# aleju/cat-generator

Measured on AMD Instinct MI355X. Metric: images/sec per G+D step, G32up-c 32x32 RGB bs=128 per GPU, higher is better.
Workload: dtype f32

## Files before the change

cat-generator_amd/csrc/common.h:

```cpp
#pragma once
#include <hip/hip_runtime.h>
#include <algorithm>
#include <stdint.h>
#include <stdio.h>
#include <string.h>
#include "../../include/catgan.h"

namespace cg {

char* err_buf();
int fail(const char* fmt, ...);

inline hipStream_t S(void* s) { return reinterpret_cast<hipStream_t>(s); }

#define CG_HIP(call)                                                              \
    do {                                                                          \
        hipError_t e__ = (call);                                                  \
        if (e__ != hipSuccess)                                                    \
            return cg::fail("%s:%d %s -> %s", __FILE__, __LINE__, #call,          \
                            hipGetErrorString(e__));                              \
    } while (0)

#define CG_LAUNCH_CHECK()                                                         \
    do {                                                                          \
        hipError_t e__ = hipGetLastError();                                       \
        if (e__ != hipSuccess)                                                    \
            return cg::fail("%s:%d kernel launch -> %s", __FILE__, __LINE__,      \
                            hipGetErrorString(e__));                              \
    } while (0)

#define CG_REQUIRE(cond, ...)                                                     \
    do {                                                                          \
        if (!(cond)) return cg::fail(__VA_ARGS__);                                \
    } while (0)

constexpr int kNumCU = 256;

#ifndef CG_TIMING_PROBE
#define CG_TIMING_PROBE 0
#endif
#define CG_PROBE_HALF(fam, T) (((CG_TIMING_PROBE) & (fam)) ? ((T) + 1) / 2 : (T))
constexpr int kEwWgsPerCU = 4, kColReduceWgsPerCU = 1;

enum Opt {
    OPT_SKINNY, OPT_GEMM_BK32, OPT_WINO_BK, OPT_NN_TILE, OPT_TN_TILE, OPT_NN_SPLITS, OPT_TN_SPLITS,
    OPT_XCD_SWIZZLE, OPT_NN_GLDS, OPT_TN_GLDS, OPT_WINO_GLDS, OPT_PAD_SKIP, OPT_WINO3, OPT_COUNT
};
long opt(Opt o);

static inline int cdiv(long a, long b) { return (int)((a + b - 1) / b); }

constexpr size_t kColScratchBytes = 8u << 20;
void* col_scratch(hipStream_t stream);
hipStream_t queue_stream(hipStream_t ref, int cls, int slot);
int queue_class(hipStream_t ref, hipStream_t s);
void wgrad_discard_all();

constexpr int kSkinnyWgradBlocks = 512;
bool skinny_ok(int ngroups, int Cin, int Cout, int kH, int kW, int padH, int padW, int ups);
size_t skinny_wgrad_ws_bytes(int Cin, int Cout);
void skinny_valu_forward(hipStream_t st, const float* x, const float* w, const float* bias, float* y, int N, int H, int W, int Cin, int Cout);
void skinny_valu_wgrad(hipStream_t st, const float* x, const float* dy, float* part, float* bias_part, int N, int H, int W, int Cin, int Cout,
                       int blocks, long ppb);
bool skinny_mfma_ok(int Cin, int Cout, int H, int W);
int skinny_mfma_forward(hipStream_t st, const float* x, const float* w, const float* bias, float* y, int N, int H, int W, int Cin, int Cout);
int skinny_mfma_wgrad(hipStream_t st, const float* x, const float* dy, float* part, float* bias_part, int N, int H, int W, int Cin, int Cout,
                      int max_blocks);

bool head_wgrad_ok(int N, int T, int C, int Co);
int head_wgrad(hipStream_t st, const float* x, const float* dy, float* gw, float* gb, int N, int T, int C, int Co, float scale);
bool wino3_geom_ok(int ngroups, int N, int H, int W, int Cin, int Cout, int kH, int kW, int padH, int padW, int ups);
int wino3_note_pack(hipStream_t st, int n, const float* const* w, float* const* wf, float* const* wb, const int* Cout, const int* Cin,
                    const int* kH, const int* kW, const int* wb_map);
int wino3_forward(hipStream_t st, int ngroups, const float* const* x, const float* const* wpk, const float* const* bias, float* const* y,
                  int N, int H, int W);

static inline int ew_grid(long n, int per_block = 256) {
    long b = (n + per_block - 1) / per_block;
    if (b < 1) b = 1;
    const long cap = (long)kNumCU * kEwWgsPerCU;
    if (b > cap) b = cap;
    return (int)b;
}

__device__ __forceinline__ float u01(uint64_t seed, uint64_t ctr) {
    uint64_t z = seed + (ctr + 1) * 0x9E3779B97F4A7C15ull;
    z = (z ^ (z >> 30)) * 0xBF58476D1CE4E5B9ull;
    z = (z ^ (z >> 27)) * 0x94D049BB133111EBull;
    z = z ^ (z >> 31);
    return (float)(z >> 40) * (1.0f / 16777216.0f);
}
__device__ __forceinline__ float wave_sum(float v) {
#pragma unroll
    for (int off = 32; off > 0; off >>= 1) v += __shfl_down(v, off, 64);
    return v;
}
__device__ __forceinline__ double wave_sum(double v) {
#pragma unroll
    for (int off = 32; off > 0; off >>= 1) v += __shfl_down(v, off, 64);
    return v;
}

#ifndef CG_COL_HANDOVER
#define CG_COL_HANDOVER 3
#endif
__device__ __forceinline__ void st_agent(double* p, double v) {
#if CG_COL_HANDOVER == 4
    const unsigned long long old = __hip_atomic_exchange((unsigned long long*)p, (unsigned long long)__double_as_longlong(v),
                                                         __ATOMIC_RELAXED, __HIP_MEMORY_SCOPE_AGENT);
    asm volatile("" ::"v"(old));
#else
    __hip_atomic_store(p, v, __ATOMIC_RELAXED, __HIP_MEMORY_SCOPE_AGENT);
#endif
}
__device__ __forceinline__ double ld_agent(const double* p) {
#if CG_COL_HANDOVER == 4
    unsigned long long zero = 0ull;
    asm volatile("" : "+v"(zero));
    return __longlong_as_double((long long)__hip_atomic_fetch_or((unsigned long long*)const_cast<double*>(p), zero, __ATOMIC_RELAXED,
                                                                 __HIP_MEMORY_SCOPE_AGENT));
#else
    return __hip_atomic_load(const_cast<double*>(p), __ATOMIC_RELAXED, __HIP_MEMORY_SCOPE_AGENT);
#endif
}

__device__ __forceinline__ bool last_block_arrives(unsigned* counter, unsigned total) {
    __shared__ int last_flag;
#if CG_COL_HANDOVER == 0
    __threadfence();
#else
    asm volatile("s_waitcnt vmcnt(0)" ::: "memory");
#endif
    __syncthreads();
    if (threadIdx.x == 0) {
#if CG_COL_HANDOVER == 3
        __builtin_amdgcn_fence(__ATOMIC_RELEASE, "agent");
#endif
// ... 70 lines not shown
```

cat-generator_amd/csrc/ops.hip:

```cpp
#include "common.h"
#include <stdarg.h>
#include <stdlib.h>
#include <algorithm>

namespace cg {
char* err_buf() {
    static thread_local char buf[512] = {0};
    return buf;
}
int fail(const char* fmt, ...) {
    va_list ap;
    va_start(ap, fmt);
    vsnprintf(err_buf(), 512, fmt, ap);
    va_end(ap);
    return 1;
}

namespace {
struct OptDef { const char* name; long dflt; };
const OptDef kOptDefs[OPT_COUNT] = {
    {"CG_SKINNY", 1}, {"CG_GEMM_BK32", 1}, {"CG_WINO_BK", 0}, {"CG_NN_TILE", 0}, {"CG_TN_TILE", 0}, {"CG_NN_SPLITS", 0}, {"CG_TN_SPLITS", 0},
    {"CG_XCD_SWIZZLE", 7}, {"CG_NN_GLDS", 1}, {"CG_TN_GLDS", 1}, {"CG_WINO_GLDS", 1}, {"CG_PAD_SKIP", 20}, {"CG_WINO3", 1},
};
long g_opt_val[OPT_COUNT];
int g_opt_state[OPT_COUNT];
}

}
#include <chrono>
#include <mutex>
#include <unordered_map>
#include <vector>
namespace cg {
void* col_scratch(hipStream_t stream) {
    constexpr int kPool = 8, kReserve = 4;
    static std::unordered_map<hipStream_t, void*> blocks;
    static std::vector<void*> pool;
    static std::mutex mu;
    std::lock_guard<std::mutex> lk(mu);
    auto it = blocks.find(stream);
    if (it != blocks.end()) return it->second;
    hipStreamCaptureStatus st = hipStreamCaptureStatusNone;
    const bool capturing = stream && hipStreamIsCapturing(stream, &st) == hipSuccess && st != hipStreamCaptureStatusNone;
    if (capturing && pool.empty()) {
        cg::fail("column reduce: no scratch block left for a stream first used inside a graph capture (run one pass on it before cg_graph_begin)");
        return nullptr;
    }
    if (!capturing && (int)pool.size() <= kReserve) {
        char* p = nullptr;
        hipStreamCaptureMode mode = hipStreamCaptureModeRelaxed;
        (void)hipThreadExchangeStreamCaptureMode(&mode);
        const bool ok = hipMalloc((void**)&p, kColScratchBytes * kPool) == hipSuccess &&
                        hipMemsetAsync(p, 0, kColScratchBytes * kPool, stream) == hipSuccess &&
                        hipStreamSynchronize(stream) == hipSuccess;
        (void)hipThreadExchangeStreamCaptureMode(&mode);
        if (!ok) {
            (void)hipGetLastError();
            if (pool.empty()) { cg::fail("column reduce: cannot allocate %zu bytes of scratch", kColScratchBytes * kPool); return nullptr; }
        } else
            for (int i = kPool - 1; i >= 0; --i) pool.insert(pool.begin(), p + (size_t)i * kColScratchBytes);
    }
    void* blk = pool.back();
    pool.pop_back();
    blocks[stream] = blk;
    return blk;
}
namespace {
__global__ void queue_probe_spin_k(unsigned long long ticks, int* sink) {
    const unsigned long long t0 = wall_clock64();
    while (wall_clock64() - t0 < ticks) { }
    if (ticks == ~0ull) *sink = 1;
}
struct QueuePool {
    std::vector<hipStream_t> s;
    std::unordered_map<hipStream_t, std::vector<int>> cls;
// ... 37 lines not shown
    std::vector<hipStream_t> rep;
    for (size_t i = 0; i < p.s.size(); ++i) {
        if (same_queue(ref, p.s[i])) { c[i] = 0; continue; }
        for (size_t k = 0; k < rep.size() && c[i] < 0; ++k)
            if (same_queue(rep[k], p.s[i])) c[i] = (int)k + 1;
        if (c[i] < 0) { rep.push_back(p.s[i]); c[i] = (int)rep.size(); }
    }
    (void)hipGetLastError();
    p.cls[ref] = c;
    return 0;
}

hipStream_t queue_stream(hipStream_t ref, int cls, int slot) {
    QueuePool& p = qpool();
    std::lock_guard<std::mutex> lk(p.mu);
    if (!p.cls.count(ref) && queue_classify(ref)) return nullptr;
    const std::vector<int>& c = p.cls[ref];
    int nclass = 0;
    for (int v : c) nclass = std::max(nclass, v + 1);
    if (nclass < 2) {
        static bool warned = false;
        if (!warned) { warned = true; fprintf(stderr, "cg: the hardware-queue probe found one queue only - side streams are plain pool streams (overlap not guaranteed)\n"); }
        return p.s[(size_t)((cls & 3) * (kQueuePool / 4) + slot % (kQueuePool / 4)) % p.s.size()];
    }
    cls = cls % nclass;
    int seen = 0;
    hipStream_t last = nullptr;
    for (size_t i = 0; i < c.size(); ++i)
        if (c[i] == cls) { last = p.s[i]; if (seen++ == slot) return p.s[i]; }
    if (last) return last;
    cg::fail("queue_stream: no pool stream on hardware queue class %d", cls);
    return nullptr;
}

int queue_class(hipStream_t ref, hipStream_t s) {
    if (s == ref) return 0;
    QueuePool& p = qpool();
    std::lock_guard<std::mutex> lk(p.mu);
    auto it = p.cls.find(ref);
    if (it == p.cls.end()) return -1;
    for (size_t i = 0; i < p.s.size(); ++i) if (p.s[i] == s) return it->second[i];
    return -1;
}

unsigned long g_opt_epoch = 1;
long opt(Opt o) {
    if (g_opt_state[o] == 0) {
        const char* e = getenv(kOptDefs[o].name);
        g_opt_val[o] = e ? atol(e) : kOptDefs[o].dflt;
        g_opt_state[o] = 1;
    }
    return g_opt_val[o];
}
}

namespace {
using cg::block_sum_256;
using cg::last_block_arrives;
using cg::wave_sum;

#define GRID_STRIDE(i, n) \
    for (long i = blockIdx.x * (long)blockDim.x + threadIdx.x; i < (n); i += (long)gridDim.x * blockDim.x)

enum { CS_RGB = 0, CS_Y = 1, CS_YUV = 2, CS_HSL = 3 };
__device__ __forceinline__ void store_colorspace(float* dst, long i, float r, float g, float b, int cs) {
#pragma clang fp contract(off)
    if (cs == CS_RGB) { dst[3 * i] = r; dst[3 * i + 1] = g; dst[3 * i + 2] = b; }
    else if (cs == CS_Y) {
        const float t0 = 0.21f * r, t1 = 0.72f * g, t2 = 0.07f * b;
        dst[i] = (t0 + t1) + t2;
    } else if (cs == CS_YUV) {
        const float y0 = 0.299f * r, y1 = 0.587f * g, y2 = 0.114f * b;
        const float u0 = -0.14713f * r, u1 = 0.28886f * g, u2 = 0.436f * b;
        const float v0 = 0.615f * r, v1 = 0.51499f * g, v2 = 0.10001f * b;
        dst[3 * i] = (y0 + y1) + y2; dst[3 * i + 1] = (u0 - u1) + u2; dst[3 * i + 2] = (v0 - v1) - v2;
    } else {
        const float mx = fmaxf(r, fmaxf(g, b)), mn = fminf(r, fminf(g, b));
        const float sum = mx + mn, l = __fdiv_rn(sum, 2.f);
        float h = 0.f, s = 0.f;
        if (mx != mn) {
            const float d = mx - mn;
            s = l > 0.5f ? __fdiv_rn(d, (2.f - mx) - mn) : __fdiv_rn(d, sum);
            if (mx == r) h = __fdiv_rn(g - b, d) + (g < b ? 6.f : 0.f);
            else if (mx == g) h = __fdiv_rn(b - r, d) + 2.f;
            else h = __fdiv_rn(r - g, d) + 4.f;
            h = __fdiv_rn(h, 6.f);
        }
        dst[3 * i] = h; dst[3 * i + 1] = s; dst[3 * i + 2] = l;
    }
}
__device__ __forceinline__ float hsl_hue(float p, float q, float t) {
#pragma clang fp contract(off)
    const float sixth = (float)(1.0 / 6.0), two_thirds = (float)(2.0 / 3.0);
    if (t < 0.f) t += 1.f;
    if (t > 1.f) t -= 1.f;
    if (t < sixth) { const float a = (q - p) * 6.f, m = a * t; return p + m; }
    if (t < 0.5f) return q;
    if (t < two_thirds) { const float a = (q - p) * (two_thirds - t), m = a * 6.f; return p + m; }
    return p;
}
__device__ __forceinline__ void colorspace_to_rgb(float a, float b, float c, int cs, float* rgb) {
#pragma clang fp contract(off)
    if (cs == CS_YUV) {
        const float rv = 1.13983f * c, gu = 0.39465f * b, gv = 0.58060f * c, bu = 2.03211f * b;
        rgb[0] = a + rv; rgb[1] = (a - gu) - gv; rgb[2] = a + bu;
    } else {
// ... 1749 lines not shown
```

cat-generator_amd/csrc/wino3.hip:

```cpp
#include "common.h"
#include <mutex>
#include <unordered_map>

namespace {

typedef float f32x16 __attribute__((ext_vector_type(16)));
typedef unsigned int u32x4 __attribute__((ext_vector_type(4)));
typedef float f32x4 __attribute__((ext_vector_type(4)));
constexpr int C = 64;
constexpr int PLD = 68;
constexpr int PW = 18, PH = 10;
constexpr int kUFloats = 16 * C * C;

__device__ __forceinline__ float4 ld4(const float* p) { return *reinterpret_cast<const float4*>(p); }
__device__ __forceinline__ float4 bufld4(__amdgpu_buffer_rsrc_t r, unsigned voff, int soff) {
    const u32x4 v = __builtin_amdgcn_raw_buffer_load_b128(r, voff, soff, 0);
    const f32x4 f = __builtin_bit_cast(f32x4, v);
    return make_float4(f.x, f.y, f.z, f.w);
}

struct PackJobs { const float* w[8]; float* uf[8]; float* ub[8]; int n; };
__global__ void wino3_pack_k(PackJobs jobs) {
    const float* __restrict__ w = jobs.w[blockIdx.y];
    const int idx = blockIdx.x * 256 + threadIdx.x;
    const int co = idx / C, ci = idx % C;
    const float G[4][3] = {{1.f, 0.f, 0.f}, {.5f, .5f, .5f}, {.5f, -.5f, .5f}, {0.f, 0.f, 1.f}};
    for (int flip = 0; flip < 2; ++flip) {
        float* U = flip ? jobs.ub[blockIdx.y] : jobs.uf[blockIdx.y];
        if (!U) continue;
        float g[3][3];
        for (int a = 0; a < 3; ++a)
            for (int b = 0; b < 3; ++b) g[a][b] = flip ? w[((long)ci * C + co) * 9 + (2 - a) * 3 + (2 - b)] : w[((long)co * C + ci) * 9 + a * 3 + b];
        float t[4][3];
        for (int i = 0; i < 4; ++i)
            for (int b = 0; b < 3; ++b) t[i][b] = G[i][0] * g[0][b] + G[i][1] * g[1][b] + G[i][2] * g[2][b];
        for (int i = 0; i < 4; ++i)
            for (int k = 0; k < 4; ++k)
                U[(((long)(i * 4 + k) * (C / 4) + ci / 4) * C + co) * 4 + (ci & 3)] = t[i][0] * G[k][0] + t[i][1] * G[k][1] + t[i][2] * G[k][2];
    }
}

constexpr int tile_of_row_c(int l) {
    return ((l < 4 || (l >= 12 && l < 16) || (l >= 20 && l < 28)) ? 0 : 16) +
           ((l < 4 || (l >= 12 && l < 16) || (l >= 20 && l < 28)) ? (l < 4 ? l : (l < 16 ? l - 8 : l - 12)) : (l < 12 ? l - 4 : (l < 20 ? l - 8 : l - 16)));
}
__device__ __forceinline__ int tile_of_row(int l) {
    const bool ga = l < 4 || (l >= 12 && l < 16) || (l >= 20 && l < 28);
    const int rank = ga ? (l < 4 ? l : (l < 16 ? l - 8 : l - 12)) : (l < 12 ? l - 4 : (l < 20 ? l - 8 : l - 16));
    return (ga ? 0 : 16) + rank;
}

template <int XI>
__device__ __forceinline__ void wino_row(const float* P, int tyl, int txl, int h, __amdgpu_buffer_rsrc_t rsU, unsigned uvoff, f32x16 (&T)[2]) {
    constexpr int I1 = XI == 0 ? 0 : (XI == 2 ? 2 : 1), I2 = XI == 0 ? 2 : (XI == 1 ? 2 : (XI == 2 ? 1 : 3));
    constexpr bool PLUS = XI == 1;
    const float* pt = P + ((2 * tyl) * PW + 2 * txl) * PLD;
    const float* r1 = pt + I1 * PW * PLD + ((h ^ ((tyl + (I1 >> 1)) & 1)) << 2);
    const float* r2 = pt + I2 * PW * PLD + ((h ^ ((tyl + (I2 >> 1)) & 1)) << 2);
    f32x16 acc[4];
#pragma unroll
    for (int k = 0; k < 4; ++k)
#pragma unroll
        for (int r = 0; r < 16; ++r) acc[k][r] = 0.f;
#pragma unroll 2
    for (int s = 0; s < CG_PROBE_HALF(8, 8); ++s) {
        float4 e[4];
#pragma unroll
        for (int c = 0; c < 4; ++c) {
            const float4 d1 = ld4(r1 + c * PLD + 8 * s), d2 = ld4(r2 + c * PLD + 8 * s);
            e[c].x = PLUS ? d1.x + d2.x : d1.x - d2.x; e[c].y = PLUS ? d1.y + d2.y : d1.y - d2.y;
            e[c].z = PLUS ? d1.z + d2.z : d1.z - d2.z; e[c].w = PLUS ? d1.w + d2.w : d1.w - d2.w;
        }
        float4 v[4], ua[4];
#pragma unroll
        for (int nu = 0; nu < 4; ++nu) {
            constexpr int J1[4] = {0, 1, 2, 1}, J2[4] = {2, 2, 1, 3};
            const float4 a = e[J1[nu]], b = e[J2[nu]];
            if (nu == 1) { v[nu].x = a.x + b.x; v[nu].y = a.y + b.y; v[nu].z = a.z + b.z; v[nu].w = a.w + b.w; }
            else { v[nu].x = a.x - b.x; v[nu].y = a.y - b.y; v[nu].z = a.z - b.z; v[nu].w = a.w - b.w; }
            ua[nu] = bufld4(rsU, uvoff, (((XI * 4 + nu) * 16 + 2 * s) * C) * 16);
        }
#define CG_W3_MF(comp) \
    _Pragma("unroll") for (int nu = 0; nu < 4; ++nu) acc[nu] = __builtin_amdgcn_mfma_f32_32x32x2f32(v[nu].comp, ua[nu].comp, acc[nu], 0, 0, 0);
        CG_W3_MF(x) CG_W3_MF(y) CG_W3_MF(z) CG_W3_MF(w)
#undef CG_W3_MF
    }
#pragma unroll
    for (int r = 0; r < 16; ++r) { T[0][r] = (acc[0][r] + acc[1][r]) + acc[2][r]; T[1][r] = (acc[1][r] - acc[2][r]) - acc[3][r]; }
}

struct W3Args {
    const float* x[4]; const float* u[4]; const float* bias[4]; float* y[4];
    int N, H, W;
};

__global__ __launch_bounds__(512, 2) void wino3_fused_k(W3Args a) {
    __shared__ __attribute__((aligned(16))) float P[PH * PW * PLD];
    const int tid = threadIdx.x, lane = tid & 63, wave = __builtin_amdgcn_readfirstlane(tid >> 6);
    const int j = lane & 31, h = lane >> 5;
    const int xi = wave & 3, nt = wave >> 2;
    const int grp = blockIdx.y;
    const float* __restrict__ x = a.x[grp];
    const float* __restrict__ U = a.u[grp];
// ... 141 lines not shown
```

cat-generator_amd/csrc/winograd.hip:

```cpp
#include "common.h"
#include <algorithm>
#include <type_traits>
#include <stdlib.h>

namespace {

typedef float f32x16 __attribute__((ext_vector_type(16)));

__device__ __forceinline__ float4 ld4(const float* p) { return *reinterpret_cast<const float4*>(p); }
__device__ __forceinline__ float wf4c(const float4& v, int i) { return i == 0 ? v.x : (i == 1 ? v.y : (i == 2 ? v.z : v.w)); }
__device__ __forceinline__ float4 f4add(float4 a, float4 b) { return make_float4(a.x + b.x, a.y + b.y, a.z + b.z, a.w + b.w); }
__device__ __forceinline__ float4 f4sub(float4 a, float4 b) { return make_float4(a.x - b.x, a.y - b.y, a.z - b.z, a.w - b.w); }

template <int MODE>
__global__ __launch_bounds__(256) void wino_input_transform_kernel(const float* __restrict__ src, float* __restrict__ V,
                                                                   int N, int Hl, int Wl, int C, int Cs) {
    const int cq_n = C >> 2;
    const int tH = Hl >> 1, tW = Wl >> 1;
    const long T = (long)N * tH * tW;
    const long total = T * cq_n;
    for (long idx = blockIdx.x * 256L + threadIdx.x; idx < total; idx += gridDim.x * 256L) {
        const int cq = (int)(idx % cq_n);
        const long tile = idx / cq_n;
        const int tj = (int)(tile % tW);
// ... 498 lines not shown
#pragma unroll
        for (int r = 0; r < 16; ++r) accM[r] = 0.f;
    }

    const int pa = a.so == 2 ? (phase >> 1) : 0, pb = a.so == 2 ? (phase & 1) : 0;
    float st1 = 0.f, st2 = 0.f;
    const float bcol = a.bias ? a.bias[n0 + wn0 + l31] : 0.f;
    if (a.lg_tw >= 0) {
        const __amdgpu_buffer_rsrc_t ry = __builtin_amdgcn_make_buffer_rsrc((void*)yout, 0, 0x7fffffff, 0x00020000);
        const int colb = (n0 + wn0 + l31) * 4;
        const int rowp = a.Wo * a.Nc * 4;
        int soffs[4];
#pragma unroll
        for (int o = 0; o < 4; ++o) soffs[o] = ((o >> 1) * a.so) * rowp + ((o & 1) * a.so) * a.Nc * 4;
#pragma unroll
        for (int r = 0; r < 16; ++r) {
            const int m = m0 + wm0 + (r & 3) + 8 * (r >> 2) + 4 * h;
            const int tj = m & (a.tW - 1), ti = (m >> a.lg_tw) & (a.tH - 1), n = m >> (a.lg_tw + a.lg_th);
            const int oy = 2 * ti * a.so + pa, ox = 2 * tj * a.so + pb;
            const unsigned vo = m < a.T ? (unsigned)(((n * a.Ho + oy) * a.Wo + ox) * a.Nc * 4 + colb) : 0x80000000u;
#pragma unroll
            for (int o = 0; o < 4; ++o) {
                const float v = accY[o][r] + bcol;
                __builtin_amdgcn_raw_buffer_store_b32(__float_as_uint(v), ry, (int)vo, soffs[o], 0);
                if (a.stats && m < a.T) { st1 += v; st2 += v * v; }
            }
        }
    } else
#pragma unroll
    for (int r = 0; r < 16; ++r) {
        const int m = m0 + wm0 + (r & 3) + 8 * (r >> 2) + 4 * h;
        if (m >= a.T) continue;
        const int tj = m % a.tW;
        const int ti = (m / a.tW) % a.tH;
        const long n = m / (a.tW * a.tH);
#pragma unroll
        for (int o = 0; o < 4; ++o) {
            const int oy = (2 * ti + (o >> 1)) * a.so + pa, ox = (2 * tj + (o & 1)) * a.so + pb;
            const float v = accY[o][r] + bcol;
            yout[((n * a.Ho + oy) * (long)a.Wo + ox) * a.Nc + n0 + wn0 + l31] = v;
            if (a.stats) { st1 += v; st2 += v * v; }
        }
    }
    if (a.stats) {
        const int srow = (phase * (int)((a.T + BM - 1) / BM) + tm) * 2 + (wave & 1);
        const float t1 = st1 + __shfl_xor(st1, 32, 64), t2 = st2 + __shfl_xor(st2, 32, 64);
        if (h == 0) {
            a.stats[((long)srow * 2 + 0) * a.Nc + n0 + wn0 + l31] = t1;
            a.stats[((long)srow * 2 + 1) * a.Nc + n0 + wn0 + l31] = t2;
        }
    }
}

__global__ __launch_bounds__(256) void wino_dy_transform_kernel(const float* __restrict__ dy, float* __restrict__ Mdy, int N,
                                                                int Hl, int Wl, int Cout, float* __restrict__ bpart) {
    const int C = 4 * Cout, cq_n = C >> 2;
    float4 bacc = make_float4(0.f, 0.f, 0.f, 0.f);
    const int tH = Hl >> 1, tW = Wl >> 1;
    const long T = (long)N * tH * tW;
    const long total = T * cq_n;
    for (long idx = blockIdx.x * 256L + threadIdx.x; idx < total; idx += gridDim.x * 256L) {
        const int cq = (int)(idx % cq_n);
        const long tile = idx / cq_n;
        const int tj = (int)(tile % tW);
        const int ti = (int)((tile / tW) % tH);
        const long n = tile / ((long)tW * tH);
        const int p = (cq * 4) / Cout, co = cq * 4 - p * Cout;
        const int pa = p >> 1, pb = p & 1;
        float4 e[2][2];
#pragma unroll
        for (int u = 0; u < 2; ++u)
#pragma unroll
            for (int v = 0; v < 2; ++v)
                e[u][v] = ld4(dy + ((n * 2 * Hl + 2 * (2 * ti + u) + pa) * (long)(2 * Wl) + 2 * (2 * tj + v) + pb) * Cout + co);
        bacc = f4add(bacc, f4add(f4add(e[0][0], e[0][1]), f4add(e[1][0], e[1][1])));
        float4 r[4][2];
#pragma unroll
        for (int v = 0; v < 2; ++v) {
            r[0][v] = e[0][v];
            r[1][v] = f4add(e[0][v], e[1][v]);
            r[2][v] = f4sub(e[0][v], e[1][v]);
            r[3][v] = make_float4(-e[1][v].x, -e[1][v].y, -e[1][v].z, -e[1][v].w);
        }
        float* out = Mdy + tile * C + cq * 4;
        const long xs = T * C;
#pragma unroll
        for (int xy = 0; xy < 4; ++xy) {
            *reinterpret_cast<float4*>(out + (xy * 4 + 0) * xs) = r[xy][0];
            *reinterpret_cast<float4*>(out + (xy * 4 + 1) * xs) = f4add(r[xy][0], r[xy][1]);
            *reinterpret_cast<float4*>(out + (xy * 4 + 2) * xs) = f4sub(r[xy][0], r[xy][1]);
            *reinterpret_cast<float4*>(out + (xy * 4 + 3) * xs) = make_float4(-r[xy][1].x, -r[xy][1].y, -r[xy][1].z, -r[xy][1].w);
        }
    }
    if (bpart) {
        __shared__ float4 shb[256];
        shb[threadIdx.x] = bacc;
        __syncthreads();
        const int cq = (int)((blockIdx.x * 256L + threadIdx.x) % cq_n);
        if (cq_n >= 256) *reinterpret_cast<float4*>(bpart + (long)blockIdx.x * C + cq * 4) = bacc;
        else if ((int)threadIdx.x < cq_n) {
            float4 t = shb[threadIdx.x];
            for (int j = threadIdx.x + cq_n; j < 256; j += cq_n) t = f4add(t, shb[j]);
            *reinterpret_cast<float4*>(bpart + (long)blockIdx.x * C + cq * 4) = t;
        }
    }
}
// ... 201 lines not shown
    }
    return 0;
}

int cg_conv2d_ups2_wino22_forward_stats(void* stream, const float* x_lo, const float* u22, const float* bias, float* y, float* v,
                                        int N, int Hp, int Wp, int Cin, int Cout, float* stats) {
    CG_REQUIRE(x_lo && u22 && y && v, "cg_conv2d_ups2_wino22_forward: null pointer");
    CG_REQUIRE(cg_conv2d_ups2_wino22_supported(N, Hp, Wp, Cin, Cout), "cg_conv2d_ups2_wino22_forward: unsupported dimensions / options");
    const int T = N * (Hp / 2) * (Wp / 2);
    hipLaunchKernelGGL(wino22_input_transform_kernel, dim3(cg::ew_grid((long)T * (Cin / 4))), dim3(256), 0, cg::S(stream), x_lo, v, N, Hp, Wp, Cin);
    CG_LAUNCH_CHECK();
    return wino_gemm_launch(stream, v, u22, bias, y, N, Hp, Wp, Cin, Cout, 0, stats, 9);
}

static int wino22_dgrad_slices(int N, int Hp, int Wp, int Cin, int Cout) {
    if (Cout % 64 != 0) return 1;
    return (long)cg::cdiv(N * (Hp / 2) * (Wp / 2), 64) * (Cin / 128) < cg::kNumCU ? 4 : 1;
}

extern "C++" template <int S>
__global__ __launch_bounds__(256) void wino22_sum_kernel(const float* __restrict__ part, float* __restrict__ out, long n4, long stride) {
    for (long i = blockIdx.x * 256L + threadIdx.x; i < n4; i += gridDim.x * 256L) {
        const float4 a = ld4(part + 4 * i), b = ld4(part + stride + 4 * i);
        float4 r = f4add(a, b);
        if (S == 4) r = f4add(r, f4add(ld4(part + 2 * stride + 4 * i), ld4(part + 3 * stride + 4 * i)));
        *reinterpret_cast<float4*>(out + 4 * i) = r;
    }
}

size_t cg_conv2d_ups2_wino22_dgrad_v_floats(int N, int Hp, int Wp, int Cin, int Cout) {
    const size_t T = (size_t)N * (Hp / 2) * (Wp / 2);
    const int sl = wino22_dgrad_slices(N, Hp, Wp, Cin, Cout);
    return 36 * T * Cout + (sl > 1 ? (size_t)sl * 4 * T * Cin : 0);
}

int cg_conv2d_ups2_wino22_dgrad(void* stream, const float* dy, const float* u_bwd, float* dx_lo, float* v_dy, int N, int Hp, int Wp, int Cin,
                                int Cout) {
    CG_REQUIRE(dy && u_bwd && dx_lo && v_dy, "cg_conv2d_ups2_wino22_dgrad: null pointer");
    CG_REQUIRE(cg_conv2d_ups2_wino22_dgrad_supported(N, Hp, Wp, Cin, Cout), "cg_conv2d_ups2_wino22_dgrad: unsupported dimensions / options");
    const int T = N * (Hp / 2) * (Wp / 2);
    hipLaunchKernelGGL(wino22_dy_input_transform_kernel, dim3(cg::ew_grid((long)T * Cout)), dim3(256), 0, cg::S(stream), dy, v_dy, N, Hp, Wp, Cout);
    CG_LAUNCH_CHECK();
    const int sl = wino22_dgrad_slices(N, Hp, Wp, Cin, Cout);
    if (sl == 1) return wino_gemm_launch(stream, v_dy, u_bwd, nullptr, dx_lo, N, Hp, Wp, Cin, Cout, 1, nullptr, 9);
    float* part = v_dy + (size_t)36 * T * Cout;
    if (wino_gemm_launch(stream, v_dy, u_bwd, nullptr, part, N, Hp, Wp, Cin, Cout, 1, nullptr, 9, sl)) return 1;
    const long n = (long)T * 4 * Cin;
    if (sl == 4) hipLaunchKernelGGL(wino22_sum_kernel<4>, dim3(cg::ew_grid(n / 4)), dim3(256), 0, cg::S(stream), part, dx_lo, n / 4, n);
    else hipLaunchKernelGGL(wino22_sum_kernel<2>, dim3(cg::ew_grid(n / 4)), dim3(256), 0, cg::S(stream), part, dx_lo, n / 4, n);
    CG_LAUNCH_CHECK();
    return 0;
}

int cg_conv2d_ups2_wino_dgrad(void* stream, const float* dy, const float* u_bwd, float* dx_lo, float* v_dy, int N, int Hp,
                              int Wp, int Cin, int Cout) {
    CG_REQUIRE(dy && u_bwd && dx_lo && v_dy, "cg_conv2d_ups2_wino_dgrad: null pointer");
    CG_REQUIRE(wino_dims_ok(N, Hp, Wp, Cin, Cout), "cg_conv2d_ups2_wino_dgrad: unsupported dimensions");
    hipStream_t st = cg::S(stream);
    const int T = N * (Hp / 2) * (Wp / 2);
    hipLaunchKernelGGL(wino_input_transform_kernel<1>, dim3(cg::ew_grid((long)T * Cout)), dim3(256), 0, st, dy, v_dy, N, Hp, Wp,
                       4 * Cout, Cout);
    CG_LAUNCH_CHECK();
    return cg_conv2d_ups2_wino_gemm(stream, v_dy, u_bwd, nullptr, dx_lo, N, Hp, Wp, Cin, Cout, 1);
}

static int wino_dgrad_slices(int N, int Hp, int Wp, int Cin, int Cout) {
    const int force = 0;
    const long T = (long)N * (Hp / 2) * (Wp / 2);
    const bool glds = cg::opt(cg::OPT_WINO_GLDS) != 0 && T * 4L * Cout * 4L < 0x7fffffffL &&
                      16L * 4L * Cout * Cin * 4L < 0x7fffffffL;
    if (!glds || !wino_dims_ok(N, Hp, Wp, Cin, Cout)) return 1;
    const long wgs = (long)cg::cdiv((int)T, 64) * (Cin / 128);
    int sl = force == 1 || force == 2 || force == 4 ? force : (wgs >= cg::kNumCU ? 1 : (wgs * 2 >= cg::kNumCU ? 2 : 4));
    while (sl > 1 && (4 * Cout / sl) % 64 != 0) sl >>= 1;
    return sl;
}
size_t cg_conv2d_ups2_wino_dgrad_part_floats(int N, int Hp, int Wp, int Cin, int Cout) {
    const int sl = wino_dgrad_slices(N, Hp, Wp, Cin, Cout);
    return sl > 1 ? (size_t)sl * N * Hp * Wp * Cin : 0;
}
int cg_conv2d_ups2_wino_dgrad_split(void* stream, const float* dy, const float* u_bwd, float* dx_lo, float* v_dy, float* part, int N, int Hp,
                                    int Wp, int Cin, int Cout) {
    const int sl = wino_dgrad_slices(N, Hp, Wp, Cin, Cout);
    if (sl <= 1 || !part) return cg_conv2d_ups2_wino_dgrad(stream, dy, u_bwd, dx_lo, v_dy, N, Hp, Wp, Cin, Cout);
    CG_REQUIRE(dy && u_bwd && dx_lo && v_dy, "cg_conv2d_ups2_wino_dgrad_split: null pointer");
    const int T = N * (Hp / 2) * (Wp / 2);
    hipLaunchKernelGGL(wino_input_transform_kernel<1>, dim3(cg::ew_grid((long)T * Cout)), dim3(256), 0, cg::S(stream), dy, v_dy, N, Hp, Wp, 4 * Cout, Cout);
    CG_LAUNCH_CHECK();
    if (wino_gemm_launch(stream, v_dy, u_bwd, nullptr, part, N, Hp, Wp, Cin, Cout, 1, nullptr, 16, sl)) return 1;
    const long n = (long)T * 4 * Cin;
    if (sl == 4) hipLaunchKernelGGL(wino22_sum_kernel<4>, dim3(cg::ew_grid(n / 4)), dim3(256), 0, cg::S(stream), part, dx_lo, n / 4, n);
    else hipLaunchKernelGGL(wino22_sum_kernel<2>, dim3(cg::ew_grid(n / 4)), dim3(256), 0, cg::S(stream), part, dx_lo, n / 4, n);
    CG_LAUNCH_CHECK();
    return 0;
}

static size_t wino_align(size_t b) { return (b + 255) / 256 * 256; }

size_t cg_conv2d_ups2_wino_wgrad_workspace_bytes(int N, int Hp, int Wp, int Cin, int Cout) {
    if (!wino_dims_ok(N, Hp, Wp, Cin, Cout)) return 0;
    const size_t T = (size_t)N * (Hp / 2) * (Wp / 2);
    return wino_align(16 * T * 4 * Cout * sizeof(float)) + wino_align((size_t)16 * 4 * Cout * Cin * sizeof(float)) +
           wino_align(std::max(sizeof(double) * Cout, (size_t)cg::kNumCU * 8 * 4 * Cout * sizeof(float))) +

           cg_conv2d_wgrad_workspace_bytes_strided(16, (int)T, 1, 1, Cin, 4 * Cout, 1, 1, 0, 0, 0);
}

int cg_conv2d_ups2_wino_wgrad(void* stream, const float* v, const float* dy, float* gw_canonical, float* gb, int N, int Hp,
                              int Wp, int Cin, int Cout, float scale, void* ws, size_t ws_bytes) {
    CG_REQUIRE(v && dy && gw_canonical, "cg_conv2d_ups2_wino_wgrad: null pointer");
    CG_REQUIRE(wino_dims_ok(N, Hp, Wp, Cin, Cout), "cg_conv2d_ups2_wino_wgrad: unsupported dimensions");
// ... 39 lines not shown
```

Before: 22810.

## Fuse Winograd dgrad input transform into GEMM kernel for upsample conv

Adds a fused kernel that loads raw dy patches into LDS via direct buffer-to-LDS loads and applies the Winograd input transform on the fly before the MFMA accumulation. The output transform is done in the epilogue through an LDS exchange across waves. This replaces a separate input-transform kernel plus GEMM, removing the write and reread of the transformed dy buffer and one launch. It applies only when tiles divide evenly and the grid covers all CUs, and it adds heavy LDS use with 512-thread blocks.

Result: faster. 23150 (median of 6 runs) (+1.5%).

```diff
diff --git a/cat-generator_amd/csrc/common.h b/cat-generator_amd/csrc/common.h
--- a/cat-generator_amd/csrc/common.h
+++ b/cat-generator_amd/csrc/common.h
@@ -44,9 +44,11 @@
 
 enum Opt {
     OPT_SKINNY, OPT_GEMM_BK32, OPT_WINO_BK, OPT_NN_TILE, OPT_TN_TILE, OPT_NN_SPLITS, OPT_TN_SPLITS,
-    OPT_XCD_SWIZZLE, OPT_NN_GLDS, OPT_TN_GLDS, OPT_WINO_GLDS, OPT_PAD_SKIP, OPT_WINO3, OPT_COUNT
+    OPT_XCD_SWIZZLE, OPT_NN_GLDS, OPT_TN_GLDS, OPT_WINO_GLDS, OPT_PAD_SKIP, OPT_WINO3, OPT_WINO_DGRAD_FUSE, OPT_WINO_DGRAD_FUSE_LAUNCHES,
+    OPT_COUNT
 };
 long opt(Opt o);
+void opt_count(Opt o);
 
 static inline int cdiv(long a, long b) { return (int)((a + b - 1) / b); }
 
@@ -83,6 +85,15 @@
     return (int)b;
 }
 
+constexpr int tile_of_row_c(int l) {
+    return ((l < 4 || (l >= 12 && l < 16) || (l >= 20 && l < 28)) ? 0 : 16) +
+           ((l < 4 || (l >= 12 && l < 16) || (l >= 20 && l < 28)) ? (l < 4 ? l : (l < 16 ? l - 8 : l - 12)) : (l < 12 ? l - 4 : (l < 20 ? l - 8 : l - 16)));
+}
+__device__ __forceinline__ int tile_of_row(int l) {
+    const bool ga = l < 4 || (l >= 12 && l < 16) || (l >= 20 && l < 28);
+    const int rank = ga ? (l < 4 ? l : (l < 16 ? l - 8 : l - 12)) : (l < 12 ? l - 4 : (l < 20 ? l - 8 : l - 16));
+    return (ga ? 0 : 16) + rank;
+}
 __device__ __forceinline__ float u01(uint64_t seed, uint64_t ctr) {
     uint64_t z = seed + (ctr + 1) * 0x9E3779B97F4A7C15ull;
     z = (z ^ (z >> 30)) * 0xBF58476D1CE4E5B9ull;
diff --git a/cat-generator_amd/csrc/ops.hip b/cat-generator_amd/csrc/ops.hip
--- a/cat-generator_amd/csrc/ops.hip
+++ b/cat-generator_amd/csrc/ops.hip
@@ -21,6 +21,7 @@
 const OptDef kOptDefs[OPT_COUNT] = {
     {"CG_SKINNY", 1}, {"CG_GEMM_BK32", 1}, {"CG_WINO_BK", 0}, {"CG_NN_TILE", 0}, {"CG_TN_TILE", 0}, {"CG_NN_SPLITS", 0}, {"CG_TN_SPLITS", 0},
     {"CG_XCD_SWIZZLE", 7}, {"CG_NN_GLDS", 1}, {"CG_TN_GLDS", 1}, {"CG_WINO_GLDS", 1}, {"CG_PAD_SKIP", 20}, {"CG_WINO3", 1},
+    {"CG_WINO_DGRAD_FUSE", 1}, {"CG_WINO_DGRAD_FUSE_LAUNCHES", 0},
 };
 long g_opt_val[OPT_COUNT];
 int g_opt_state[OPT_COUNT];
@@ -164,6 +165,7 @@
     }
     return g_opt_val[o];
 }
+void opt_count(Opt o) { opt(o); ++g_opt_val[o]; }
 }
 
 namespace {
diff --git a/cat-generator_amd/csrc/wino3.hip b/cat-generator_amd/csrc/wino3.hip
--- a/cat-generator_amd/csrc/wino3.hip
+++ b/cat-generator_amd/csrc/wino3.hip
@@ -40,15 +40,8 @@
     }
 }
 
-constexpr int tile_of_row_c(int l) {
-    return ((l < 4 || (l >= 12 && l < 16) || (l >= 20 && l < 28)) ? 0 : 16) +
-           ((l < 4 || (l >= 12 && l < 16) || (l >= 20 && l < 28)) ? (l < 4 ? l : (l < 16 ? l - 8 : l - 12)) : (l < 12 ? l - 4 : (l < 20 ? l - 8 : l - 16)));
-}
-__device__ __forceinline__ int tile_of_row(int l) {
-    const bool ga = l < 4 || (l >= 12 && l < 16) || (l >= 20 && l < 28);
-    const int rank = ga ? (l < 4 ? l : (l < 16 ? l - 8 : l - 12)) : (l < 12 ? l - 4 : (l < 20 ? l - 8 : l - 16));
-    return (ga ? 0 : 16) + rank;
-}
+using cg::tile_of_row;
+using cg::tile_of_row_c;
 
 template <int XI>
 __device__ __forceinline__ void wino_row(const float* P, int tyl, int txl, int h, __amdgpu_buffer_rsrc_t rsU, unsigned uvoff, f32x16 (&T)[2]) {
diff --git a/cat-generator_amd/csrc/winograd.hip b/cat-generator_amd/csrc/winograd.hip
--- a/cat-generator_amd/csrc/winograd.hip
+++ b/cat-generator_amd/csrc/winograd.hip
@@ -574,6 +574,217 @@
     }
 }
 
+struct WinoFusedArgs {
+    const float* dy;
+    const float* U;
+    float* y;
+    int N, tH, tW, Cs, K, Nc;
+    int bH, bW;
+    int xcd;
+};
+constexpr int kFusedPatchSlots = 18 * 18 * 8;
+constexpr int kFusedPatchInstr = (kFusedPatchSlots + 63) / 64;
+constexpr int kFusedPatchFloats = kFusedPatchInstr * 64 * 4;
+constexpr int kFusedUFloats = 16 * 8 * 64;
+
+__device__ __forceinline__ int fused_pidx(int px) { return (px >> 1) + 9 * (px & 1); }
+__device__ __forceinline__ int fused_swz(int py, int px) { return (((px >> 2) & 3) << 1) | ((py >> 1) & 1); }
+
+__global__ __launch_bounds__(512, 2) void wino_dgrad_fused_kernel(WinoFusedArgs a) {
+    __shared__ __attribute__((aligned(16))) float P0[kFusedPatchFloats];
+    __shared__ __attribute__((aligned(16))) float P1[kFusedPatchFloats];
+    __shared__ __attribute__((aligned(16))) float U0[kFusedUFloats];
+    __shared__ __attribute__((aligned(16))) float U1[kFusedUFloats];
+    const int tid = threadIdx.x, lane = tid & 63, wave = __builtin_amdgcn_readfirstlane(tid >> 6);
+    const int j = lane & 31, h = lane >> 5;
+    const int xy = wave & 3, mh = wave >> 2;
+    const int Hl = 2 * a.tH, Wl = 2 * a.tW;
+    const int ncb = a.Nc >> 6, nblk = a.N * a.bH * a.bW;
+    int cb = blockIdx.x % ncb, blk = blockIdx.x / ncb;
+    if (a.xcd && (nblk & 7) == 0) {
+        const int slot = blockIdx.x >> 3;
+        cb = slot % ncb;
+        blk = (slot / ncb) * 8 + (blockIdx.x & 7);
+    }
+    const int bx = blk % a.bW, by = (blk / a.bW) % a.bH, n = blk / (a.bW * a.bH);
+    const int ty0 = by * 8, tx0 = bx * 8, n0 = cb * 64;
+
+    const unsigned img_bytes = (unsigned)(4 * Hl * Wl * a.Cs) * 4u;
+    const __amdgpu_buffer_rsrc_t rsd = __builtin_amdgcn_make_buffer_rsrc((void*)(a.dy + (long)n * 4 * Hl * Wl * a.Cs), 0, img_bytes, 0x00020000);
+    const __amdgpu_buffer_rsrc_t rsu = __builtin_amdgcn_make_buffer_rsrc((void*)a.U, 0, 0x7fffffff, 0x00020000);
+    constexpr int PJ = (kFusedPatchInstr + 7) / 8;
+    unsigned pvoff[PJ];
+#pragma unroll
+    for (int jj = 0; jj < PJ; ++jj) {
+        const int slot = (wave + 8 * jj) * 64 + lane;
+        const int pi = slot >> 3, py = pi / 18, pxi = pi - py * 18;
+        const int px = pxi < 9 ? 2 * pxi : 2 * (pxi - 9) + 1;
+        const int q = (slot & 7) ^ fused_swz(py, px);
+        const int iy = 2 * ty0 - 1 + py, ix = 2 * tx0 - 1 + px;
+        const bool in = slot < kFusedPatchSlots && iy >= 0 && iy < Hl && ix >= 0 && ix < Wl;
+        pvoff[jj] = in ? (unsigned)(((2 * iy * 2 * Wl + 2 * ix) * a.Cs + 4 * q) * 4) : 0x80000000u;
+    }
+    unsigned uvoff[4];
+#pragma unroll
+    for (int i = 0; i < 4; ++i) {
+        const int idx = wave * 4 + i, pos = idx >> 1, kh = idx & 1;
+        uvoff[i] = (unsigned)(((pos * a.K + kh * 4 + (lane >> 4)) * a.Nc + n0 + 4 * (lane & 15)) * 4);
+    }
+    auto dma_patch = [&](auto pbc, auto partc, int kp) {
+        constexpr int PB = decltype(pbc)::value, PART = decltype(partc)::value;
+        constexpr int J0 = PART == 0 ? 0 : (PART == 1 ? 2 : (PART == 2 ? 4 : 5)), J1 = PART == 0 ? 2 : (PART == 1 ? 4 : (PART == 2 ? 5 : 6));
+        const int k0 = kp * 32, p = k0 / a.Cs, cs0 = k0 - p * a.Cs;
+        const int soff = (((p >> 1) * 2 * Wl + (p & 1)) * a.Cs + cs0) * 4;
+#pragma unroll
+        for (int jj = J0; jj < J1 && jj < PJ; ++jj)
+            if (wave + 8 * jj < kFusedPatchInstr) wino_glds16(rsd, (PB ? P1 : P0) + (wave + 8 * jj) * 256, pvoff[jj], soff);
+    };
+    auto dma_u = [&](auto ubc, int k) {
+        constexpr int UB = decltype(ubc)::value;
+        const int soff = k * a.Nc * 4;
+#pragma unroll
+        for (int i = 0; i < 4; ++i) wino_glds16(rsu, (UB ? U1 : U0) + (wave * 4 + i) * 256, uvoff[i], soff);
+    };
+
+    const int I1 = xy == 0 ? 0 : (xy == 2 ? 2 : 1), I2 = xy == 0 ? 2 : (xy == 1 ? 2 : (xy == 2 ? 1 : 3));
+    const int tl = cg::tile_of_row(j), tyl = (tl >> 3) + 4 * mh, txl = tl & 7;
+    int pa_rd[2][4];
+#pragma unroll
+    for (int rr = 0; rr < 2; ++rr)
+#pragma unroll
+        for (int c = 0; c < 4; ++c) {
+            const int py = 2 * tyl + (rr ? I2 : I1), px = 2 * txl + c;
+            pa_rd[rr][c] = ((py * 18 + fused_pidx(px)) * 8 + (h ^ fused_swz(py, px))) * 16;
+        }
+    const float sgn = xy == 1 ? 1.f : -1.f;
+    const int ub_rd = xy * 4 * 512 + h * 4 * 64 + j;
+
+    f32x16 acc[4][2];
+#pragma unroll
+    for (int nu = 0; nu < 4; ++nu)
+#pragma unroll
+        for (int ni = 0; ni < 2; ++ni)
+#pragma unroll
+            for (int r = 0; r < 16; ++r) acc[nu][ni][r] = 0.f;
+
+    using I0c = std::integral_constant<int, 0>;
+    using I1c = std::integral_constant<int, 1>;
+    using I2c = std::integral_constant<int, 2>;
+    using I3c = std::integral_constant<int, 3>;
+    const int KP = CG_PROBE_HALF(4, a.K / 32);
+    dma_patch(I0c{}, I0c{}, 0); dma_patch(I0c{}, I1c{}, 0); dma_patch(I0c{}, I2c{}, 0); dma_patch(I0c{}, I3c{}, 0);
+    dma_u(I0c{}, 0);
+    asm volatile("s_waitcnt vmcnt(0)" ::: "memory");
+    __syncthreads();
+
+    auto sub_step = [&](auto pbc, auto sc, int kp) {
+        constexpr int PB = decltype(pbc)::value, S = decltype(sc)::value;
+        const bool more_p = kp + 1 < KP;
+        if (more_p) dma_patch(std::integral_constant<int, PB ^ 1>{}, sc, kp + 1);
+        if (S < 3 || more_p) dma_u(std::integral_constant<int, (S & 1) ^ 1>{}, kp * 32 + 8 * S + 8);
+        const char* P = reinterpret_cast<const char*>(PB ? P1 : P0);
+        const float* B = ((S & 1) ? U1 : U0) + ub_rd;
+        float4 d1[4], d2[4];
+#pragma unroll
+        for (int c = 0; c < 4; ++c) {
+            d1[c] = *reinterpret_cast<const float4*>(P + (pa_rd[0][c] ^ (S << 5)));
+            d2[c] = *reinterpret_cast<const float4*>(P + (pa_rd[1][c] ^ (S << 5)));
+        }
+        auto frag = [&](int comp, float (&o)[4]) {
+            float e[4];
+#pragma unroll
+            for (int c = 0; c < 4; ++c) e[c] = __builtin_fmaf(sgn, wf4c(d2[c], comp), wf4c(d1[c], comp));
+            o[0] = e[0] - e[2]; o[1] = e[1] + e[2]; o[2] = e[2] - e[1]; o[3] = e[1] - e[3];
+        };
+        float b[2][8], v[2][4];
+#pragma unroll
+        for (int i = 0; i < 8; ++i) b[0][i] = B[(i >> 1) * 512 + (i & 1) * 32];
+        frag(0, v[0]);
+#pragma unroll
+        for (int comp = 0; comp < 4; ++comp) {
+            if (comp < 3) {
+#pragma unroll
+                for (int i = 0; i < 8; ++i) b[(comp + 1) & 1][i] = B[(i >> 1) * 512 + (comp + 1) * 64 + (i & 1) * 32];
+                frag(comp + 1, v[(comp + 1) & 1]);
+            }
+            __builtin_amdgcn_sched_barrier(0);
+#pragma unroll
+            for (int i = 0; i < 8; ++i)
+                acc[i >> 1][i & 1] = __builtin_amdgcn_mfma_f32_32x32x2f32(v[comp & 1][i >> 1], b[comp & 1][i], acc[i >> 1][i & 1], 0, 0, 0);
+            __builtin_amdgcn_sched_barrier(0);
+        }
+        asm volatile("s_waitcnt vmcnt(0)" ::: "memory");
+        __syncthreads();
+    };
+    for (int kp = 0; kp < KP; kp += 2) {
+        sub_step(I0c{}, I0c{}, kp); sub_step(I0c{}, I1c{}, kp); sub_step(I0c{}, I2c{}, kp); sub_step(I0c{}, I3c{}, kp);
+        sub_step(I1c{}, I0c{}, kp + 1); sub_step(I1c{}, I1c{}, kp + 1); sub_step(I1c{}, I2c{}, kp + 1); sub_step(I1c{}, I3c{}, kp + 1);
+    }
+
+    static_assert(kFusedPatchFloats >= 8 * 1024, "the epilogue's exchange fits in a patch buffer");
+    const __amdgpu_buffer_rsrc_t rsy = __builtin_amdgcn_make_buffer_rsrc((void*)(a.y + (long)n * Hl * Wl * a.Nc), 0, (unsigned)(Hl * Wl * a.Nc) * 4u, 0x00020000);
+    const int rowb = 2 * Wl * a.Nc * 4, colb = 2 * a.Nc * 4;
+    float* const X = mh ? P1 : P0;
+    auto store_out = [&](int o, int ni, const f32x16& Y) {
+        const int lane_base = (((2 * ty0 + (o >> 1)) * Wl + 2 * tx0 + (o & 1)) * a.Nc + n0 + ni * 32 + j) * 4;
+#pragma unroll
+        for (int r = 0; r < 16; ++r) {
+            const int row0 = (r & 3) + 8 * (r >> 2);
+            const int t = h ? cg::tile_of_row_c(row0 + 4) : cg::tile_of_row_c(row0);
+            const int ty = (t >> 3) + 4 * mh, tx = t & 7;
+            const bool in = ty0 + ty < a.tH && tx0 + tx < a.tW;
+            const unsigned vo = in ? (unsigned)(lane_base + ty * rowb + tx * colb) : 0x80000000u;
+            __builtin_amdgcn_raw_buffer_store_b32(__float_as_uint(Y[r] + 0.f), rsy, (int)vo, 0, 0);
+        }
+    };
+    const float cyr[2] = {xy < 3 ? 1.f : 0.f, xy == 0 ? 0.f : (xy == 1 ? 1.f : -1.f)};
+    auto add_row = [&](int o, int ni, f32x16& Y) {
+        const bool first = (o >> 1) == 0 ? xy == 0 : xy == 1;
+        float* Xo = X + (o * 2 + ni) * 1024;
+#pragma unroll
+        for (int r = 0; r < 16; ++r) Y[r] = first ? 0.f : Xo[r * 64 + lane];
+#pragma unroll
+        for (int xx = 0; xx < 4; ++xx) {
+            const float cx = (o & 1) == 0 ? (xx < 3 ? 1.f : 0.f) : (xx == 0 ? 0.f : (xx == 1 ? 1.f : -1.f));
+            const float c = cyr[o >> 1] * cx;
+            if (c != 0.f) {
+#pragma unroll
+                for (int r = 0; r < 16; ++r) Y[r] += c * acc[xx][ni][r];
+            }
+        }
+    };
+#pragma unroll
+    for (int row = 0; row < 4; ++row) {
+        if (xy == row) {
+#pragma unroll
+            for (int o = 0; o < 4; ++o) {
+                if (cyr[o >> 1] == 0.f) continue;
+#pragma unroll
+                for (int ni = 0; ni < 2; ++ni) {
+                    f32x16 Y;
+                    add_row(o, ni, Y);
+                    if (row == 3) store_out(o, ni, Y);
+                    else {
+                        float* Xo = X + (o * 2 + ni) * 1024;
+#pragma unroll
+                        for (int r = 0; r < 16; ++r) Xo[r * 64 + lane] = Y[r];
+                    }
+                }
+            }
+        } else if (row == 3 && xy < 2) {
+#pragma unroll
+            for (int ni = 0; ni < 2; ++ni) {
+                f32x16 Y;
+                const float* Xo = X + (xy * 2 + ni) * 1024;
+#pragma unroll
+                for (int r = 0; r < 16; ++r) Y[r] = Xo[r * 64 + lane];
+                if (xy == 0) store_out(0, ni, Y); else store_out(1, ni, Y);
+            }
+        }
+        if (row < 3) __syncthreads();
+    }
+}
+
 __global__ __launch_bounds__(256) void wino_dy_transform_kernel(const float* __restrict__ dy, float* __restrict__ Mdy, int N,
                                                                 int Hl, int Wl, int Cout, float* __restrict__ bpart) {
     const int C = 4 * Cout, cq_n = C >> 2;
@@ -881,11 +1092,33 @@
     return 0;
 }
 
+static bool wino_dgrad_fused_takes(const float* dy, const float* u_bwd, const float* dx_lo, int N, int Hp, int Wp, int Cin, int Cout) {
+    const long mode = cg::opt(cg::OPT_WINO_DGRAD_FUSE);
+    if (mode == 0) return false;
+    const int tH = Hp / 2, tW = Wp / 2, bH = cg::cdiv(tH, 8), bW = cg::cdiv(tW, 8);
+    const long wgs = (long)N * bH * bW * (Cin / 64);
+    const bool fits = 4L * Hp * Wp * Cout * 4L < 0x7fffffffL && (long)Hp * Wp * Cin * 4L < 0x7fffffffL && 16L * 4L * Cout * Cin * 4L < 0x7fffffffL &&
+                      Cout % 32 == 0 && Cin % 64 == 0 && wgs <= 0x7fffffffL &&
+                      ((uintptr_t)dy % 16) == 0 && ((uintptr_t)u_bwd % 16) == 0 && ((uintptr_t)dx_lo % 4) == 0;
+    if (!fits) return false;
+    return mode == 2 || (tH % 8 == 0 && tW % 8 == 0 && wgs >= cg::kNumCU);
+}
+
 int cg_conv2d_ups2_wino_dgrad(void* stream, const float* dy, const float* u_bwd, float* dx_lo, float* v_dy, int N, int Hp,
                               int Wp, int Cin, int Cout) {
     CG_REQUIRE(dy && u_bwd && dx_lo && v_dy, "cg_conv2d_ups2_wino_dgrad: null pointer");
     CG_REQUIRE(wino_dims_ok(N, Hp, Wp, Cin, Cout), "cg_conv2d_ups2_wino_dgrad: unsupported dimensions");
     hipStream_t st = cg::S(stream);
+    if (wino_dgrad_fused_takes(dy, u_bwd, dx_lo, N, Hp, Wp, Cin, Cout)) {
+        WinoFusedArgs f;
+        f.dy = dy; f.U = u_bwd; f.y = dx_lo; f.N = N; f.tH = Hp / 2; f.tW = Wp / 2; f.Cs = Cout; f.K = 4 * Cout; f.Nc = Cin;
+        f.bH = cg::cdiv(f.tH, 8); f.bW = cg::cdiv(f.tW, 8);
+        f.xcd = (int)cg::opt(cg::OPT_XCD_SWIZZLE);
+        hipLaunchKernelGGL(wino_dgrad_fused_kernel, dim3((unsigned)(N * f.bH * f.bW * (Cin / 64))), dim3(512), 0, st, f);
+        CG_LAUNCH_CHECK();
+        cg::opt_count(cg::OPT_WINO_DGRAD_FUSE_LAUNCHES);
+        return 0;
+    }
     const int T = N * (Hp / 2) * (Wp / 2);
     hipLaunchKernelGGL(wino_input_transform_kernel<1>, dim3(cg::ew_grid((long)T * Cout)), dim3(256), 0, st, dy, v_dy, N, Hp, Wp,
                        4 * Cout, Cout);
```
